# dgrzech/sobfu

Hardware: AMD Instinct MI355X
Metric: solver iterations/sec on 256^3 voxel grid (higher is better)
Workload: dtype f32

## Files before the change

include/sobfu_hip.h:

```cpp
#ifndef SOBFU_HIP_H
#define SOBFU_HIP_H

#include <stddef.h>
#include <stdint.h>

#if defined(__GNUC__)
#pragma GCC visibility push(default)
#endif
#ifdef __cplusplus
extern "C" {
#endif

#define SOBFU_HIP_ABI_VERSION 3

#define SOBFU_E_BADARG (-1)
#define SOBFU_E_FILTER (-2)
#define SOBFU_E_UNSUPPORTED (-3)

int sobfu_hip_abi_version(void);
const char* sobfu_hip_error_string(int code);

int sobfu_hip_clear_volume(float* d_vol, int X, int Y, int Z, void* stream);
int sobfu_hip_integrate_depth(const float* d_dists, int dists_step_bytes, int rows, int cols, float* d_vol, int X,
                              int Y, int Z, const float voxel_size[3], float trunc_dist, float eta,
// ... 10 lines not shown
int sobfu_hip_init_plane(float* d_vol, int X, int Y, int Z, const float voxel_size[3], float trunc_dist, float z,
                         void* stream);
int sobfu_hip_init_torus(float* d_vol, int X, int Y, int Z, const float voxel_size[3], float trunc_dist,
                         const float t[2], void* stream);

int sobfu_hip_bilateral_filter(const uint16_t* d_src, int src_step_bytes, uint16_t* d_dst, int dst_step_bytes,
                               int rows, int cols, int kernel_size, float sigma_spatial, float sigma_depth,
                               void* stream);
int sobfu_hip_truncate_depth(uint16_t* d_depth, int step_bytes, int rows, int cols, float max_dist_m, void* stream);
int sobfu_hip_compute_dists(const uint16_t* d_depth, int depth_step_bytes, float* d_dists, int dists_step_bytes,
                            int rows, int cols, float fx, float fy, float cx, float cy, void* stream);

int sobfu_hip_clear_field(float* d_field, int X, int Y, int Z, void* stream);
int sobfu_hip_init_identity(float* d_psi, int X, int Y, int Z, void* stream);
int sobfu_hip_apply(const float* d_phi, float* d_phi_warped, const float* d_psi, int X, int Y, int Z, void* stream);
int sobfu_hip_estimate_inverse(const float* d_psi, float* d_psi_inv, int X, int Y, int Z, int n_sweeps,
                               void* stream);
int sobfu_hip_inverse_and_warp(const float* d_psi, float* d_psi_inv, const float* d_phi, float* d_phi_warped, int X, int Y, int Z,
                               int n_sweeps, void* stream);
int sobfu_hip_tsdf_gradient(const float* d_vol, float* d_grad, int X, int Y, int Z, void* stream);
int sobfu_hip_laplacian(const float* d_psi, float* d_L, int X, int Y, int Z, void* stream);
int sobfu_hip_jacobian(const float* d_psi, float* d_J, int X, int Y, int Z, int mode, void* stream);
int sobfu_hip_clear_jacobian(float* d_J, int X, int Y, int Z, void* stream);

int sobfu_hip_sobolev_filter(int s, float lambda, float* out);
int sobfu_hip_potential_gradient(const float* d_phi_n_psi, const float* d_phi_global, const float* d_grad,
                                 const float* d_L, float* d_nabla_U, float w_reg, int X, int Y, int Z, void* stream);
int sobfu_hip_convolution_rows(float* d_dst, const float* d_src, const float taps[7], int w, int h, int d,
                               void* stream);
int sobfu_hip_convolution_columns(float* d_dst, const float* d_src, const float taps[7], int w, int h, int d,
                                  void* stream);
int sobfu_hip_convolution_depth(float* d_dst, const float* d_src, const float taps[7], int w, int h, int d,
                                void* stream);
int sobfu_hip_update_psi(float* d_psi, const float* d_nabla_U_S, float* d_updates, float alpha, int X, int Y, int Z,
                         void* stream);

int sobfu_hip_reduce_config(int n, int* blocks, int* threads);
int sobfu_hip_data_energy(const float* d_phi_global, const float* d_phi_n, int n, void* d_scratch, float* out,
                          void* stream);
int sobfu_hip_reg_energy_sobolev(const float* d_J, int n, void* d_scratch, float* out, void* stream);
int sobfu_hip_max_update_norm(const float* d_updates, int n, void* d_scratch, float out[2], void* stream);
int sobfu_hip_reg_energy_sobolev_from_psi(const float* d_psi, int X, int Y, int Z, void* d_scratch, float* out,
                                          void* stream);

int sobfu_hip_fused_potential_gradient(const float* d_phi_n_psi, const float* d_phi_global, const float* d_psi,
                                       float* d_nabla_U, float w_reg, int X, int Y, int Z, void* stream);
int sobfu_hip_fused_smooth_update_apply(const float* d_nabla_U, float* d_psi, const float* d_phi_n,
                                        float* d_phi_n_psi, float* d_updates, uint32_t* d_max_sq_slots,
                                        const float taps[7], float alpha, int X, int Y, int Z, void* stream);

int sobfu_hip_pack_vec3(const float* d_src4, float* d_dst3, size_t n, void* stream);
int sobfu_hip_unpack_vec3(const float* d_src3, float* d_dst4, size_t n, void* stream);
int sobfu_hip_extract_tsdf(const float* d_src2, float* d_dst1, size_t n, void* stream);

int sobfu_hip_tile3_init_identity(float* d_psi, int Lx, int Ly, int Lz, int xb, int yb, int zb, void* stream);
int sobfu_hip_tile3_apply(const float* d_phi, int Xg, int Yg, int Zg, float* d_phi_warped, const float* d_psi, int Lx, int Ly, int Lz,
                          void* stream);
int sobfu_hip_tile3_estimate_inverse(const float* d_psi, int Xg, int Yg, int Zg, float* d_psi_inv, int Lx, int Ly, int Lz, int xb, int yb,
                                     int zb, int n_sweeps, void* stream);
int sobfu_hip_tile3_estimate_inverse_window(const float* d_psi_win, const int win[6], int Xg, int Yg, int Zg, float* d_psi_inv, int Lx, int Ly, int Lz,
                                            int xb, int yb, int zb, const int box[6], int n_sweeps, int* d_violation, void* stream);
int sobfu_hip_tile3_apply_window(const float* d_phi_win, const int win[6], int Xg, int Yg, int Zg, float* d_phi_warped, const float* d_psi, int Lx,
                                 int Ly, int Lz, const int box[6], int* d_violation, void* stream);
int sobfu_hip_tile3_max_displacement(const float* d_psi, int Lx, int Ly, int Lz, int xb, int yb, int zb, const int box[6], uint32_t* d_max_bits,
                                     void* stream);
int sobfu_hip_tile3_integrate_depth(const float* d_dists, int dists_step_bytes, int rows, int cols, float* d_vol_local, int Lx, int Ly,
                                    int Lz, int xb, int yb, int zb, const float voxel_size[3], float trunc_dist, float eta,
                                    const float R[9], const float t[3], float fx, float fy, float cx, float cy, void* stream);
int sobfu_hip_tile3_potential_gradient(const float* d_phi_n_psi, const float* d_phi_global, const float* d_psi, float* d_nabla_U,
                                       float w_reg, int Lx, int Ly, int Lz, const int box[6], int thin,
                                       const uint32_t* d_prev_slots, float max_update_norm, int compact, void* stream);
int sobfu_hip_tile3_smooth_update_apply(const float* d_nabla_U, float* d_psi, const float* d_phi_n, float* d_phi_n_psi, float* d_updates,
                                        uint32_t* d_max_sq_slots, const float taps[7], float alpha, int Lx, int Ly, int Lz, int Xg,
                                        int Yg, int Zg, const int own[6], const int box[6], int thin,
                                        const uint32_t* d_prev_slots, float max_update_norm, int compact, void* stream);
int sobfu_hip_tile3_apply_tsdf_only(const float* d_phi1, int Xg, int Yg, int Zg, float* d_out1, const float* d_psi3, int Lx, int Ly, int Lz,
                                    void* stream);
int sobfu_hip_tile3_pack(const float* d_field3, int Lx, int Ly, int Lz, float* d_buf, const int* boxes, int n_boxes, void* stream);
int sobfu_hip_tile3_unpack(float* d_field3, int Lx, int Ly, int Lz, const float* d_buf, const int* boxes, int n_boxes, void* stream);

typedef struct sobfu_hip_solver sobfu_hip_solver;

typedef struct {
    int verbosity;
    int max_iter;
    int s;
    float max_update_norm;
    float lambda;
    float alpha;
    float w_reg;
} sobfu_hip_solver_params;

typedef struct {
    int iterations;
    int converged;
    float last_max_update_norm;
    float last_max_update_index;
    float last_e_data, last_e_reg;
} sobfu_hip_solver_report;

int sobfu_hip_solver_create(sobfu_hip_solver** out, int X, int Y, int Z, const sobfu_hip_solver_params* params);
int sobfu_hip_solver_destroy(sobfu_hip_solver* s);
int sobfu_hip_solver_set_params(sobfu_hip_solver* s, const sobfu_hip_solver_params* params);
size_t sobfu_hip_solver_workspace_bytes(const sobfu_hip_solver* s);
int sobfu_hip_solver_estimate_psi(sobfu_hip_solver* s, const float* d_phi_global, float* d_phi_global_psi_inv,
                                  const float* d_phi_n, float* d_phi_n_psi, float* d_psi, float* d_psi_inv,
// ... 190 lines not shown
```

sobfu_amd/build_host.py:

```python
from __future__ import annotations

import os
import subprocess

HERE = os.path.dirname(os.path.abspath(__file__))
ROOT = os.path.dirname(HERE)
ROCM = os.environ.get("ROCM_PATH", "/opt/rocm")
INC = os.path.join(ROOT, "include")
CSRC = os.path.join(HERE, "csrc")
LIB = os.path.join(HERE, "libsobfu_hip.so")
SOBFU_HPP = os.path.join(INC, "sobfu_amd", "sobfu.hpp")
DEPTH_IO_HPP = os.path.join(INC, "sobfu_amd", "depth_io.hpp")
SOBFU_HIP_H = os.path.join(INC, "sobfu_hip.h")
EVALUATE_HPP = os.path.join(INC, "sobfu_amd", "evaluate.hpp")


def _test_src(name: str) -> str:
    return os.path.join(ROOT, "tests", "cpp", name)


def _build(out: str, src: str, deps, linked: bool, force: bool = False, flags=()) -> str:
    out = os.path.join(ROOT, "build", out)
    deps = [src, *deps] + ([LIB] if linked else [])
    if not force and os.path.exists(out) and all(os.path.getmtime(out) >= os.path.getmtime(d) for d in deps):
# ... 16 lines not shown
    return _build("depth_io_tool", _test_src("depth_io_tool.cpp"), [DEPTH_IO_HPP], False, force, ["-std=c++14", "-lz"])


def build_png_tool(force: bool = False) -> str:
    return _build("png_write_tool", _test_src("png_write_tool.cpp"), [DEPTH_IO_HPP], False, force, ["-std=c++14", "-lz"])


def build_colour_tool(force: bool = False) -> str:
    return _build("colour_io_tool", _test_src("colour_io_tool.cpp"), [DEPTH_IO_HPP, SOBFU_HPP, SOBFU_HIP_H], True, force)


def build_ply_tool(force: bool = False) -> str:
    return _build("ply_write_tool", _test_src("ply_write_tool.cpp"), [SOBFU_HPP, SOBFU_HIP_H], True, force)


def build_variant_tool(force: bool = False) -> str:
    return _build("variant_tool", _test_src("variant_tool.cpp"), [os.path.join(CSRC, "sobfu_variant.hpp"), SOBFU_HIP_H], False, force,
                  ["-std=c++17", f"-I{CSRC}"])


def build_geometry_tool(force: bool = False, flags=()) -> str:
    deps = [os.path.join(CSRC, h) for h in ("sobfu_geometry.hpp", "sobfu_tile_layout.hpp", "sobfu_variant.hpp")] + [SOBFU_HIP_H]
    return _build("geometry_tool", _test_src("geometry_tool.cpp"), deps, False, force, ["-std=c++17", f"-I{CSRC}", *flags])


def build_icp_tool(force: bool = False) -> str:
    return _build("icp_shell_tool", _test_src("icp_shell_tool.cpp"), [SOBFU_HPP], True, force)


def build_mesh_warp_tool(force: bool = False) -> str:
    return _build("mesh_warp_tool", _test_src("mesh_warp_tool.cpp"), [SOBFU_HPP, DEPTH_IO_HPP], True, force)


def build_mesh_eval_tool(force: bool = False) -> str:
    deps = [SOBFU_HPP, EVALUATE_HPP, SOBFU_HIP_H, os.path.join(CSRC, "sobfu_mesh_distance.hpp")]
    return _build("mesh_eval_tool", _test_src("mesh_eval_tool.cpp"), deps, True, force, [f"-I{CSRC}", "-ffp-contract=off"])


def build_mesh_ray_tool(force: bool = False, flags=()) -> str:
    deps = [os.path.join(CSRC, h) for h in ("sobfu_mesh_ray.hpp", "sobfu_mesh_distance.hpp")]
    return _build("mesh_ray_tool", _test_src("mesh_ray_tool.cpp"), deps, False, force, ["-std=c++14", f"-I{CSRC}", "-ffp-contract=off", *flags])


def build_mesh_parity_tool(force: bool = False, flags=()) -> str:
    deps = [os.path.join(CSRC, h) for h in ("sobfu_mesh_parity.hpp", "sobfu_mesh_distance.hpp")]
    return _build("mesh_parity_tool", _test_src("mesh_parity_tool.cpp"), deps, False, force, ["-std=c++14", f"-I{CSRC}", "-ffp-contract=off", *flags])


def build_rigid_tool(force: bool = False) -> str:
    return _build("rigid_solve_tool", _test_src("rigid_solve_tool.cpp"), [os.path.join(CSRC, "sobfu_rigid.hpp")], False, force,
                  ["-std=c++14", f"-I{CSRC}", "-ffp-contract=off"])


def build_host(force: bool = False) -> str:
    for build in (build_app, build_io_tool, build_png_tool, build_colour_tool, build_ply_tool, build_variant_tool, build_geometry_tool,
                  build_icp_tool, build_mesh_warp_tool, build_mesh_eval_tool, build_mesh_ray_tool, build_mesh_parity_tool, build_rigid_tool):
        build(force)
    return _build("host_shell_tests", _test_src("host_shell_tests.cpp"), [SOBFU_HPP, EVALUATE_HPP, SOBFU_HIP_H], True, force)


if __name__ == "__main__":
    print(build_host(force=True))
```

sobfu_amd/csrc/sobfu_launch.hpp:

```cpp
#pragma once
#include <hip/hip_runtime.h>

#include <cstddef>
#include <cstdint>

#include "sobfu_geometry.hpp"

namespace sobfu_hip {
struct PassALaunch {
    const float* pnp = nullptr;
    const float* pg  = nullptr;
    const float* psi = nullptr;
    float* nU        = nullptr;
    float w_reg      = 0.f;
    int X = 0, Y = 0, Z = 0;
    LaunchBox boxes[kMaxBoxes] = {};
    int n_boxes = 0;
    const uint32_t* prev_slots = nullptr;
    float max_update_norm      = 0.f;
    bool compact = false;
    bool warp    = false;
};
struct PassBLaunch {
    const float* nU     = nullptr;
    float* psi          = nullptr;
    float* psi_out      = nullptr;
    const float* phi_n  = nullptr;
    float* pnp          = nullptr;
    float* updates      = nullptr;
    uint32_t* slots     = nullptr;
    const float* taps   = nullptr;
    float alpha         = 0.f;
    int X = 0, Y = 0, Z = 0;
    int pX = 0, pY = 0, pZ = 0;
    int own[6] = {};
    LaunchBox boxes[kMaxBoxes] = {};
    int n_boxes = 0;
    const uint32_t* prev_slots = nullptr;
    float max_update_norm      = 0.f;
    int prev_rows = 1;
    bool compact  = false;
    bool sys_acquire = false;
    bool warp        = false;
};
inline void set_whole_grid(PassALaunch& l, int X, int Y, int Z) {
    l.X = X; l.Y = Y; l.Z = Z;
    l.boxes[0] = LaunchBox{0, X, 0, Y, 0, Z, false};
    l.n_boxes  = 1;
}
inline void set_whole_grid(PassBLaunch& l, int X, int Y, int Z) {
    l.X = X; l.Y = Y; l.Z = Z;
    l.pX = X; l.pY = Y; l.pZ = Z;
    const int own[6] = {0, X, 0, Y, 0, Z};
    for (int i = 0; i < 6; ++i) l.own[i] = own[i];
    l.boxes[0] = LaunchBox{0, X, 0, Y, 0, Z, false};
    l.n_boxes  = 1;
}
int launch_pass_a(const PassALaunch& l, hipStream_t stream);
int launch_pass_b(const PassBLaunch& l, hipStream_t stream);
constexpr int kMaxSync = 64;
struct TileSync {
    uint32_t ticket_push, reserved;
    uint64_t wait_ticks;
    uint32_t wait_count, pad0;
    uint32_t err;
    uint32_t n_sync;
    uint32_t my_rank, world;
    uint64_t timeout_ticks;
    uint32_t* my_flags;
    uint32_t* my_grows;
    int sync_rank[kMaxSync];
    uint32_t* peer_flags[kMaxSync];
    uint32_t* peer_grows[kMaxSync];
};
struct TilePassAPlan;
int tile_pass_a_plan_create(TilePassAPlan** out, const TileLaunchBox* boxes, int n, int X, int Y, int Z);
void tile_pass_a_plan_destroy(TilePassAPlan* p);
int launch_tile_pass_a_plan(const TilePassAPlan* p, const float* pnp, const float* pg, const float* psi, float* nU, float w_reg, TileSync* sync,
                            uint32_t seq, int wait, const uint32_t* row, uint32_t row_index, hipStream_t stream);
int launch_tile_flush(TileSync* sync, uint32_t seq, int wait, const uint32_t* row, uint32_t row_index, hipStream_t stream);
int launch_tile_pingpong(TileSync* sync, int q, int first, uint32_t seq0, int reps, hipStream_t stream);
int launch_pack_vec(const float* src4, float* dst3, size_t N, hipStream_t stream);
int launch_unpack_vec(const float* src3, float* dst4, size_t N, hipStream_t stream);
int launch_extract_tsdf(const float* src2, float* dst1, size_t N, hipStream_t stream);
int launch_apply_tsdf_only(const float* phi1, float* out1, const float* psi3, int X, int Y, int Z, hipStream_t stream, int phi_Z = 0, int phi_X = 0,
                           int phi_Y = 0);
int launch_msg_copy(bool pack, float* field3, float* buf, int Lx, int Ly, int Lz, const int* boxes, int n, hipStream_t stream);
int launch_msg_scatter_table(float* field3, const float* buf, const uint32_t* d_table, unsigned n_cells, hipStream_t stream);
int launch_compact_enter(const float* psi4, const float* pg2, const float* pn2, float* c_psi, float* c_g, float* c_n, float* c_f, int X, int Y,
                         int Z, hipStream_t stream);
int launch_compact_leave(const float* c_psi, const float* pn2, float* psi4, float* pnp2, int X, int Y, int Z, hipStream_t stream);
int data_energy_tsdf(const float* g1, const float* f1, int n, void* d_scratch, float* out, hipStream_t stream);
int reg_energy_from_psi3(const float* psi3, int X, int Y, int Z, void* d_scratch, float* out, hipStream_t stream);
}
```

sobfu_amd/csrc/sobfu_variant.hpp:

```cpp
#pragma once

#include <cstddef>
#include <cstdlib>

#include "sobfu_hip.h"

namespace sobfu_hip {

inline long env_cache_cells() {
    const char* e = getenv("SOBFU_CACHE_CELLS");
    return e ? atol(e) : 3300000L;
}
inline int env_pipe_b() {
    const char* e = getenv("SOBFU_PIPE_B");
    return e ? (atoi(e) != 0 ? 1 : 0) : -1;
}
inline bool env_warp_a() {
    const char* e = getenv("SOBFU_WARP_A");
    return !(e && atoi(e) == 0);
}

struct GridTraits {
    bool resident;
    bool idx32;
    bool arrays32;
    bool plane32;
    int pipe_b;
};
inline GridTraits grid_traits(int X, int Y, int Z, int pX, int pY, int pZ, long cache_cells, int pipe_b = -1) {
    const size_t n = (size_t) X * Y * Z;
    GridTraits g;
    g.resident = (long) n <= cache_cells;
    g.idx32    = (size_t) pX * pY * pZ < ((size_t) 1 << 30);
    g.arrays32 = n * 12 < ((size_t) 1 << 32);
    g.plane32  = (size_t) X * Y * 16 < ((size_t) 1 << 32);
    g.pipe_b   = pipe_b;
    return g;
}

struct PassAVariant {
    bool compact, nt, warp;
    constexpr bool operator==(const PassAVariant& o) const { return compact == o.compact && nt == o.nt && warp == o.warp; }
};
inline constexpr PassAVariant kPassATable[] = {
    {true,      true,  true},
    {true,      false, false},
    {true,      true,  false},
    {false,     false, false},
};
inline constexpr PassAVariant kTilePassATable[] = {
    {true,  false, false},
    {true,  true,  false},
    {false, false, false},
};
inline int choose_pass_a(const GridTraits& g, bool compact, bool warp, bool tile, PassAVariant* v) {
    if (warp && (tile || !compact || g.resident || !g.idx32)) return SOBFU_E_UNSUPPORTED;
    v->compact = compact;
    v->nt      = compact && !g.resident;
    v->warp    = warp;
    return 0;
}

struct PassBVariant {
    bool updates, compact, direct, idx32, lead, nt, pipe, ntbuf, apply;
    constexpr bool operator==(const PassBVariant& o) const {
        return updates == o.updates && compact == o.compact && direct == o.direct && idx32 == o.idx32 && lead == o.lead && nt == o.nt &&
               pipe == o.pipe && ntbuf == o.ntbuf && apply == o.apply;
    }
};
inline constexpr PassBVariant kPassBTable[] = {
    {true , true , true , false, false, true , false, false, true },
// ... 13 lines not shown
    {false, true , false, true , true , true , false, false, true },
    {false, true , false, true , false, false, true , false, true },
    {false, true , false, true , false, false, false, false, true },
    {false, true , false, true , false, true , true , false, true },
    {false, true , false, true , false, true , false, true , true },
    {false, true , false, true , false, true , false, false, true },
    {false, true , false, false, false, true , false, false, true },
    {false, false, false, false, false, true , false, false, true },
};
struct PassBAsk {
    bool compact, updates;
    bool sys_acquire;
    bool apply;
};
struct PassBMarch {
    bool pipe         = false;
    bool direct       = false;
    bool long_marches = false;
};
inline int pass_b_march(const GridTraits& g, const PassBAsk& k, PassBMarch* m) {
    if (!g.plane32) return SOBFU_E_UNSUPPORTED;
    if (k.sys_acquire && !g.arrays32) return SOBFU_E_UNSUPPORTED;
    m->pipe = k.compact && g.idx32 && !k.updates && g.arrays32 && (k.sys_acquire || (g.pipe_b >= 0 ? g.pipe_b != 0 : g.resident));
    if (k.sys_acquire && !m->pipe) return SOBFU_E_UNSUPPORTED;
    return 0;
}
inline int choose_pass_b(const GridTraits& g, const PassBAsk& k, const PassBMarch& m, PassBVariant* v) {
    if (!k.apply && (m.direct || !k.compact || !g.idx32 || k.updates || g.resident || m.pipe || !g.arrays32 || k.sys_acquire))
        return SOBFU_E_UNSUPPORTED;
    const bool own_format = k.compact && g.idx32 && !k.updates, plain_nt = !g.resident && !m.pipe;
    v->updates = k.updates;
    v->compact = k.compact;
    v->direct  = m.direct;
    v->idx32   = own_format;
    v->lead    = own_format && plain_nt && !m.direct && m.long_marches;
    v->nt      = !own_format || !g.resident;
    v->pipe    = own_format && m.pipe;
    v->ntbuf   = own_format && plain_nt && g.arrays32;
    v->apply   = k.apply;
    return 0;
}

inline bool loop_warps_in_pass_a(const GridTraits& g) {
    const PassBAsk b{true, false, false, false};
    PassAVariant va;
    PassBVariant vb;
    PassBMarch m;
    return choose_pass_a(g, true, true, false, &va) == 0 && pass_b_march(g, b, &m) == 0 && choose_pass_b(g, b, m, &vb) == 0;
}
inline bool loop_warps_in_pass_a(int X, int Y, int Z) {
    return env_warp_a() && loop_warps_in_pass_a(grid_traits(X, Y, Z, X, Y, Z, env_cache_cells(), env_pipe_b()));
}

}
```

sobfu_amd/csrc/solver_capi.hip:

```cpp
#include <algorithm>
#include <cmath>
#include <cstdio>
#include <cstdlib>
#include <cstring>
#include <string>
#include <vector>

#include "sobfu_device.hpp"
#include "sobfu_hip.h"
#include "sobfu_host.hpp"
#include "sobfu_launch.hpp"


namespace {

using sobfu_hip::DevicePtr;
using sobfu_hip::EventPtr;
using sobfu_hip::kSlots;
using sobfu_hip::slots_to_norm;
constexpr int kCheckEvery = 32;
constexpr int kMaxRunAhead = 96;

}

struct sobfu_hip_solver {
    int X = 0, Y = 0, Z = 0;
    size_t N = 0;
    sobfu_hip_solver_params p{};
    float taps[7]{};
    DevicePtr<float> nabla_U;
    DevicePtr<float> updates;
    DevicePtr<float> c_psi;
    DevicePtr<float> c_f;
    DevicePtr<float> c_g;
    DevicePtr<float> c_n;
    bool compact = true;
    DevicePtr<uint32_t> slots;
    sobfu_hip::PinnedPtr<uint32_t> h_rows;
    int h_rows_iters   = 0;
    EventPtr ev_chk;
    DevicePtr<void> red_scratch;
    int slots_iters    = 0;
    bool keep_updates  = false;
    sobfu_hip_log_fn log_fn = nullptr;
    void* log_user          = nullptr;
    bool log_set            = false;
    size_t bytes            = 0;
    int prof_stride = 0;
    std::vector<EventPtr> events;
    double ms_a = 0, ms_b = 0;
    int prof_launches = 0, prof_pending = 0;
    struct Session {
        bool active = false, compact = false;
        const float *pg = nullptr, *pn = nullptr;
        float *pnp = nullptr, *psi = nullptr;
        const float *it_pnp = nullptr, *it_pg = nullptr, *it_pn = nullptr;
        float *it_psi = nullptr, *it_out = nullptr, *upd = nullptr;
        int cap = 0;
        int launched = 0;
        int checked = 0, fl_to = 0;
        bool in_flight = false;
        int done = 0;
        bool converged = false;
        float last_norm = 0.f;
        bool inline_log = false;
        bool warp = false;
    } q;

    void log(const std::string& line) const {
        if (log_set) {
            if (log_fn) log_fn(line.c_str(), log_user);
        } else {
            std::printf("%s\n", line.c_str());
        }
    }
};

namespace {

std::string fmt_g(float v) {
    char b[64];
    std::snprintf(b, sizeof b, "%g", (double) v);
    return b;
}

int ensure_slots(sobfu_hip_solver* s, int iters) {
    if (iters <= s->slots_iters) return 0;
    if (s->slots) s->bytes -= (size_t) (s->slots_iters + 1) * kSlots * 4;
    s->slots_iters = 0;
    SOBFU_HIP_TRY(sobfu_hip::device_alloc(s->slots, (size_t) (iters + 1) * kSlots * 4));
    s->slots_iters = iters;
    s->bytes += (size_t) (iters + 1) * kSlots * 4;
    return 0;
}

int ensure_poll(sobfu_hip_solver* s, int iters) {
    if (!s->ev_chk) SOBFU_HIP_TRY(sobfu_hip::event_create(s->ev_chk, hipEventDisableTiming));
    if (iters <= s->h_rows_iters) return 0;
    s->h_rows.reset();
    s->h_rows_iters = 0;
    void* h = nullptr;
    SOBFU_HIP_TRY(hipHostMalloc(&h, (size_t) iters * kSlots * 4, hipHostMallocDefault));
    s->h_rows.reset((uint32_t*) h);
    s->h_rows_iters = iters;
    return 0;
}

int ensure_compact(sobfu_hip_solver* s) {
    if (s->c_psi) return 0;
    SOBFU_HIP_TRY(sobfu_hip::device_alloc(s->c_psi, s->N * 12));
    SOBFU_HIP_TRY(sobfu_hip::device_alloc(s->c_f, s->N * 4));
    SOBFU_HIP_TRY(sobfu_hip::device_alloc(s->c_g, s->N * 4));
    SOBFU_HIP_TRY(sobfu_hip::device_alloc(s->c_n, s->N * 4));
    s->bytes += s->N * 24;
    return 0;
}

int ensure_updates(sobfu_hip_solver* s) {
    if (s->updates) return 0;
    SOBFU_HIP_TRY(sobfu_hip::device_alloc(s->updates, s->N * 16));
    s->bytes += s->N * 16;
    return 0;
}

int set_params(sobfu_hip_solver* s, const sobfu_hip_solver_params* p) {
    SOBFU_CHECK_ARGS(p && p->max_iter >= 0);
    if (p->s < 7 || p->s > 16) return p->s < 7 ? SOBFU_E_UNSUPPORTED : SOBFU_E_FILTER;
    float h[16];
    SOBFU_TRY(sobfu_hip_sobolev_filter(p->s, p->lambda, h));
    for (int i = 0; i < 7; ++i) s->taps[i] = h[i];
    s->p = *p;
    return 0;
}

int ensure_events(sobfu_hip_solver* s, size_t n) {
    while (s->events.size() < n) {
        EventPtr e;
        SOBFU_HIP_TRY(sobfu_hip::event_create(e, hipEventDefault));
        s->events.push_back(std::move(e));
    }
    return 0;
}

int session_begin_impl(sobfu_hip_solver* s, const float* pg, const float* pn, float* pnp, float* psi, int cap, hipStream_t st) {
    sobfu_hip_solver::Session& q = s->q;
    const int X = s->X, Y = s->Y, Z = s->Z;
    q = sobfu_hip_solver::Session{};
    q.pg = pg; q.pn = pn; q.pnp = pnp; q.psi = psi;
    q.cap = cap;
    q.compact = s->compact && cap > 0;
    q.last_norm = NAN;
    if (!q.compact) SOBFU_TRY(sobfu_hip_apply(pn, pnp, psi, X, Y, Z, st));
    if (cap <= 0) return 0;
    SOBFU_TRY(ensure_slots(s, cap));
    SOBFU_HIP_TRY(hipMemsetAsync(s->slots.get(), 0, (size_t) (cap + 1) * kSlots * 4, st));
    if (s->keep_updates) {
        SOBFU_TRY(ensure_updates(s));
        q.upd = s->updates.get();
    }
    q.it_pnp = pnp; q.it_pg = pg; q.it_pn = pn; q.it_psi = psi; q.it_out = pnp;
    if (q.compact) {
        SOBFU_TRY(ensure_compact(s));
        SOBFU_TRY(sobfu_hip::launch_compact_enter(psi, pg, pn, s->c_psi.get(), s->c_g.get(), s->c_n.get(), s->c_f.get(), X, Y, Z, st));
        q.it_pnp = s->c_f.get(); q.it_pg = s->c_g.get(); q.it_pn = s->c_n.get(); q.it_psi = s->c_psi.get(); q.it_out = s->c_f.get();
        q.warp = s->p.verbosity == 0 && !q.upd && sobfu_hip::loop_warps_in_pass_a(X, Y, Z);
    }
    if (s->p.max_update_norm >= 0.f) SOBFU_TRY(ensure_poll(s, cap));
    if (s->prof_stride > 0) SOBFU_TRY(ensure_events(s, (size_t) 3 * (cap / s->prof_stride + 1)));
    return 0;
}
int session_begin(sobfu_hip_solver* s, const float* pg, const float* pn, float* pnp, float* psi, int cap, hipStream_t st) {
    if (s->q.active) return SOBFU_E_BADARG;
    const int rc = session_begin_impl(s, pg, pn, pnp, psi, cap, st);
    s->q.active = rc == 0;
    return rc;
}

void session_examine(sobfu_hip_solver* s, int upto, float* per_iter) {
    sobfu_hip_solver::Session& q = s->q;
    for (int k = q.checked; k < upto && !q.converged; ++k) {
        const float v = slots_to_norm(s->h_rows.get() + (size_t) k * kSlots);
        if (per_iter) per_iter[k] = v;
        q.last_norm = v;
        q.done = k + 1;
        if (v <= s->p.max_update_norm) q.converged = true;
    }
    q.checked = upto;
}

int session_enqueue(sobfu_hip_solver* s, int n, bool poll, float* per_iter, hipStream_t st) {
    sobfu_hip_solver::Session& q = s->q;
    if (!q.active || n < 0 || q.launched + n > q.cap) return SOBFU_E_BADARG;
    const int X = s->X, Y = s->Y, Z = s->Z;
    const sobfu_hip_solver_params& p = s->p;
    const bool can_converge = p.max_update_norm >= 0.f;
    const int last = q.launched + n;
    sobfu_hip::PassALaunch A;
    sobfu_hip::set_whole_grid(A, X, Y, Z);
    A.pnp = q.warp ? q.it_pn : q.it_pnp; A.pg = q.it_pg; A.psi = q.it_psi; A.nU = s->nabla_U.get(); A.w_reg = p.w_reg;
    A.max_update_norm = p.max_update_norm;
    A.compact = q.compact;
    A.warp    = q.warp;
    sobfu_hip::PassBLaunch B;
    sobfu_hip::set_whole_grid(B, X, Y, Z);
    B.nU = s->nabla_U.get(); B.psi = q.it_psi; B.phi_n = q.it_pn; B.pnp = q.it_out; B.updates = q.upd; B.taps = s->taps; B.alpha = p.alpha;
    B.max_update_norm = p.max_update_norm;
    B.compact = q.compact;
    B.warp    = q.warp;
    for (int it = q.launched + 1; it <= last && !q.converged; ++it) {
        const uint32_t* prev = (it > 1) ? s->slots.get() + (size_t) (it - 1) * kSlots : nullptr;
        uint32_t* cur        = s->slots.get() + (size_t) it * kSlots;
        const bool ev = s->prof_stride > 0 && (it % s->prof_stride == 0) && (size_t) 3 * (s->prof_pending + 1) <= s->events.size();
        const int e0  = 3 * s->prof_pending;
        if (ev) SOBFU_HIP_TRY(hipEventRecord(s->events[e0].get(), st));
        A.prev_slots = B.prev_slots = prev;
        B.slots = cur;
        SOBFU_TRY(sobfu_hip::launch_pass_a(A, st));
        if (ev) SOBFU_HIP_TRY(hipEventRecord(s->events[e0 + 1].get(), st));
        SOBFU_TRY(sobfu_hip::launch_pass_b(B, st));
        if (ev) {
            SOBFU_HIP_TRY(hipEventRecord(s->events[e0 + 2].get(), st));
            s->prof_pending += 1;
        }
        q.launched = it;
        if (can_converge && poll) {
            if (!q.in_flight && (it % kCheckEvery == 0 || it == last)) {
                SOBFU_HIP_TRY(hipMemcpyAsync(s->h_rows.get() + (size_t) q.checked * kSlots, s->slots.get() + (size_t) (q.checked + 1) * kSlots,
                                             (size_t) (it - q.checked) * kSlots * 4, hipMemcpyDeviceToHost, st));
                SOBFU_HIP_TRY(hipEventRecord(s->ev_chk.get(), st));
                q.in_flight = true;
                q.fl_to     = it;
            }
            if (q.in_flight) {
                const bool must_wait = it - q.checked >= kMaxRunAhead;
                hipError_t e = must_wait ? hipEventSynchronize(s->ev_chk.get()) : hipEventQuery(s->ev_chk.get());
                if (e == hipSuccess) {
                    session_examine(s, q.fl_to, per_iter);
                    q.in_flight = false;
                } else if (e != hipErrorNotReady) {
                    return (int) e;
                }
            }
        }
    }
    return 0;
}

int session_drain(sobfu_hip_solver* s, float* per_iter, hipStream_t st) {
    sobfu_hip_solver::Session& q = s->q;
    if (q.launched == 0) return 0;
    if (s->p.max_update_norm >= 0.f) {
        if (q.in_flight) {
            SOBFU_HIP_TRY(hipEventSynchronize(s->ev_chk.get()));
            session_examine(s, q.fl_to, per_iter);
            q.in_flight = false;
// ... 301 lines not shown
```

sobfu_amd/csrc/solver_kernels.hip:

```cpp
#include <type_traits>

#include "sobfu_device.hpp"
#include "sobfu_hip.h"
#include "sobfu_host.hpp"
#include "sobfu_launch.hpp"

using namespace sobfu_hip;

#ifndef SOBFU_SWIZZLE_B
#define SOBFU_SWIZZLE_B true
#endif

namespace {

struct Taps {
    float s[7];
};
constexpr int kMaxMsgs = 18;

#include "solver_iter_common.inl"
#include "solver_pass_a.inl"
#include "solver_pass_b.inl"
#include "solver_aux_kernels.inl"

}

namespace sobfu_hip {

template <size_t I = 0, class Row, size_t N, class F>
static bool launch_row(const Row (&table)[N], const Row& v, F&& launch) {
    if constexpr (I < N) {
        if (table[I] == v) {
            launch(std::integral_constant<size_t, I>{});
            return true;
        }
        return launch_row<I + 1>(table, v, launch);
    } else {
        return false;
    }
}

static int launch_tile_boxes(const TilePassAArgsP& a, int groups, const PassAVariant& v, hipStream_t stream) {
    const dim3 grid((unsigned) groups), block(TX, kWY);
    const bool found = launch_row(kTilePassATable, v, [&](auto i) {
        constexpr PassAVariant V = kTilePassATable[decltype(i)::value];
        hipLaunchKernelGGL((tile_potential_gradient_kernel<kRPT, kWY, V.compact, V.nt ? kNT : 0>), grid, block, 0, stream, a);
    });
    return found ? (int) hipGetLastError() : SOBFU_E_UNSUPPORTED;
}

int launch_pass_a(const PassALaunch& L, hipStream_t stream) {
    if (L.n_boxes > kMaxBoxes) return SOBFU_E_BADARG;
    const bool direct = has_direct_box(L.boxes, L.n_boxes);
    const GridTraits g = grid_traits(L.X, L.Y, L.Z, L.X, L.Y, L.Z, env_cache_cells());
    PassAVariant v;
    SOBFU_TRY(choose_pass_a(g, L.compact, L.warp, direct, &v));
    if (direct) {
        TileBoxList B{};
        const int total = plan_pass_a_thin(B, L.boxes, L.n_boxes, g.resident);
        if (total <= 0) return total < 0 ? SOBFU_E_BADARG : 0;
        TileBoxList* d = nullptr;
        SOBFU_HIP_TRY(hipMallocAsync((void**) &d, sizeof B, stream));
        const hipError_t e = hipMemcpyAsync(d, &B, sizeof B, hipMemcpyHostToDevice, stream);
        const TilePassAArgsP a{{L.pnp, L.pg, L.psi, L.nU, {L.X, L.Y, L.Z}, L.w_reg, nullptr, 0.f}, d, {nullptr, 0, 0, nullptr, 0}};
        const int rc = e != hipSuccess ? (int) e : launch_tile_boxes(a, total, v, stream);
        const hipError_t f = hipFreeAsync(d, stream);
        return rc != 0 ? rc : (int) f;
    }
    PassAArgs a{{L.pnp, L.pg, L.psi, L.nU, {L.X, L.Y, L.Z}, L.w_reg, L.prev_slots, L.max_update_norm}, {}};
    const int groups = plan_pass_a(a.boxes, L.boxes, L.n_boxes);
    if (groups == 0) return 0;
    const dim3 grid((unsigned) groups), block(TX, kWY);
    const bool found = launch_row(kPassATable, v, [&](auto i) {
        constexpr PassAVariant V = kPassATable[decltype(i)::value];
        hipLaunchKernelGGL((fused_potential_gradient_kernel<kRPT, kWY, V.compact, V.nt ? kNT : 0, V.warp>), grid, block, 0, stream, a);
    });
    return found ? (int) hipGetLastError() : SOBFU_E_UNSUPPORTED;
}

struct TilePassAPlan {
    TileBoxList* d_boxes = nullptr;
    int groups = 0, X = 0, Y = 0, Z = 0;
};
int tile_pass_a_plan_create(TilePassAPlan** out, const TileLaunchBox* boxes, int n, int X, int Y, int Z) {
    TileBoxList L{};
    const int total = fill_tile_boxes(L, boxes, n, grid_traits(X, Y, Z, X, Y, Z, env_cache_cells()).resident);
    if (total < 0) return SOBFU_E_BADARG;
    auto* p = new TilePassAPlan();
    p->groups = total; p->X = X; p->Y = Y; p->Z = Z;
    hipError_t e = hipSuccess;
    if (total > 0) {
        e = hipMalloc((void**) &p->d_boxes, sizeof L);
        if (e == hipSuccess) e = hipMemcpy(p->d_boxes, &L, sizeof L, hipMemcpyHostToDevice);
    }
    if (e != hipSuccess) {
        if (p->d_boxes) (void) hipFree(p->d_boxes);
        delete p;
        return (int) e;
    }
    *out = p;
    return 0;
}
void tile_pass_a_plan_destroy(TilePassAPlan* p) {
    if (p == nullptr) return;
    if (p->d_boxes) (void) hipFree(p->d_boxes);
    delete p;
}
int launch_tile_pass_a_plan(const TilePassAPlan* p, const float* pnp, const float* pg, const float* psi, float* nU, float w_reg, TileSync* sync,
                            uint32_t seq, int wait, const uint32_t* row, uint32_t row_index, hipStream_t stream) {
    if (p->groups == 0) return 0;
    PassAVariant v;
    SOBFU_TRY(choose_pass_a(grid_traits(p->X, p->Y, p->Z, p->X, p->Y, p->Z, env_cache_cells()), true, false, true, &v));
    const TilePassAArgsP a{{pnp, pg, psi, nU, {p->X, p->Y, p->Z}, w_reg, nullptr, 0.f}, p->d_boxes, {sync, seq, wait, row, row_index}};
    return launch_tile_boxes(a, p->groups, v, stream);
}

int launch_tile_pingpong(TileSync* sync, int q, int first, uint32_t seq0, int reps, hipStream_t stream) {
    hipLaunchKernelGGL(tile_pingpong_kernel, dim3(1), dim3(64), 0, stream, sync, q, first, seq0, reps);
    return (int) hipGetLastError();
}

int launch_tile_flush(TileSync* sync, uint32_t seq, int wait, const uint32_t* row, uint32_t row_index, hipStream_t stream) {
    hipLaunchKernelGGL(tile_flush_kernel, dim3(1), dim3(64), 0, stream, sync, seq, wait, row, row_index);
    return (int) hipGetLastError();
}

int launch_pass_b(const PassBLaunch& L, hipStream_t stream) {
    if (L.n_boxes > kMaxBoxes) return SOBFU_E_BADARG;
// ... 64 lines not shown
    return (int) hipGetLastError();
}
#undef SOBFU_LIN
int launch_compact_enter(const float* psi4, const float* pg2, const float* pn2, float* c_psi, float* c_g, float* c_n, float* c_f, int X, int Y,
                         int Z, hipStream_t stream) {
    hipLaunchKernelGGL(compact_enter_kernel, voxel_grid(X, Y, Z), voxel_block(), 0, stream, (const float4*) psi4, (const float2*) pg2,
                       (const float2*) pn2, (P3*) c_psi, c_g, c_n, c_f, Dims{X, Y, Z});
    return (int) hipGetLastError();
}
int launch_compact_leave(const float* c_psi, const float* pn2, float* psi4, float* pnp2, int X, int Y, int Z, hipStream_t stream) {
    hipLaunchKernelGGL(compact_leave_kernel, voxel_grid(X, Y, Z), voxel_block(), 0, stream, (const P3*) c_psi, (const float2*) pn2,
                       (float4*) psi4, (float2*) pnp2, Dims{X, Y, Z});
    return (int) hipGetLastError();
}

}

extern "C" {

int sobfu_hip_fused_potential_gradient(const float* d_phi_n_psi, const float* d_phi_global, const float* d_psi,
                                       float* d_nabla_U, float w_reg, int X, int Y, int Z, void* stream) {
    SOBFU_CHECK_ARGS(d_phi_n_psi && d_phi_global && d_psi && d_nabla_U && X > 1 && Y > 1 && Z > 1);
    if ((size_t) X * Y * Z > (size_t) 0x7fffffff) return SOBFU_E_UNSUPPORTED;
    sobfu_hip::PassALaunch L;
    sobfu_hip::set_whole_grid(L, X, Y, Z);
    L.pnp = d_phi_n_psi; L.pg = d_phi_global; L.psi = d_psi; L.nU = d_nabla_U; L.w_reg = w_reg;
    return sobfu_hip::launch_pass_a(L, (hipStream_t) stream);
}

int sobfu_hip_fused_smooth_update_apply(const float* d_nabla_U, float* d_psi, const float* d_phi_n, float* d_phi_n_psi,
                                        float* d_updates, uint32_t* d_max_sq_slots, const float taps[7], float alpha,
                                        int X, int Y, int Z, void* stream) {
    SOBFU_CHECK_ARGS(d_nabla_U && d_psi && d_phi_n && d_phi_n_psi && d_max_sq_slots && taps && X > 0 && Y > 0 && Z > 0);
    if ((size_t) X * Y * Z > (size_t) 0x7fffffff) return SOBFU_E_UNSUPPORTED;
    sobfu_hip::PassBLaunch L;
    sobfu_hip::set_whole_grid(L, X, Y, Z);
    L.nU = d_nabla_U; L.psi = d_psi; L.phi_n = d_phi_n; L.pnp = d_phi_n_psi; L.updates = d_updates; L.slots = d_max_sq_slots;
    L.taps = taps; L.alpha = alpha;
    return sobfu_hip::launch_pass_b(L, (hipStream_t) stream);
}

int sobfu_hip_pack_vec3(const float* d_src4, float* d_dst3, size_t n, void* stream) {
    SOBFU_CHECK_ARGS(d_src4 && d_dst3 && n > 0);
    return sobfu_hip::launch_pack_vec(d_src4, d_dst3, n, (hipStream_t) stream);
}
int sobfu_hip_unpack_vec3(const float* d_src3, float* d_dst4, size_t n, void* stream) {
    SOBFU_CHECK_ARGS(d_src3 && d_dst4 && n > 0);
    return sobfu_hip::launch_unpack_vec(d_src3, d_dst4, n, (hipStream_t) stream);
}
int sobfu_hip_extract_tsdf(const float* d_src2, float* d_dst1, size_t n, void* stream) {
    SOBFU_CHECK_ARGS(d_src2 && d_dst1 && n > 0);
    return sobfu_hip::launch_extract_tsdf(d_src2, d_dst1, n, (hipStream_t) stream);
}
static bool box_ok(const int b[6], int Lx, int Ly, int Lz) {
    return b[0] >= 0 && b[0] <= b[1] && b[1] <= Lx && b[2] >= 0 && b[2] <= b[3] && b[3] <= Ly && b[4] >= 0 && b[4] <= b[5] && b[5] <= Lz;
}

int sobfu_hip_tile3_potential_gradient(const float* d_phi_n_psi, const float* d_phi_global, const float* d_psi, float* d_nabla_U, float w_reg,
                                       int Lx, int Ly, int Lz, const int box[6], int thin, const uint32_t* d_prev_slots,
                                       float max_update_norm, int compact, void* stream) {
    SOBFU_CHECK_ARGS(d_phi_n_psi && d_phi_global && d_psi && d_nabla_U && Lx > 1 && Ly > 1 && Lz > 1 && box && box_ok(box, Lx, Ly, Lz));
    if ((size_t) Lx * Ly * Lz > (size_t) 0x7fffffff) return SOBFU_E_UNSUPPORTED;
    sobfu_hip::PassALaunch L;
    L.pnp = d_phi_n_psi; L.pg = d_phi_global; L.psi = d_psi; L.nU = d_nabla_U; L.w_reg = w_reg;
    L.X = Lx; L.Y = Ly; L.Z = Lz;
    L.boxes[0] = sobfu_hip::LaunchBox{box[0], box[1], box[2], box[3], box[4], box[5], thin != 0};
    L.n_boxes = 1;
    L.prev_slots = d_prev_slots; L.max_update_norm = max_update_norm;
    L.compact = compact != 0;
    return sobfu_hip::launch_pass_a(L, (hipStream_t) stream);
}

int sobfu_hip_tile3_smooth_update_apply(const float* d_nabla_U, float* d_psi, const float* d_phi_n, float* d_phi_n_psi, float* d_updates,
                                        uint32_t* d_max_sq_slots, const float taps[7], float alpha, int Lx, int Ly, int Lz, int Xg, int Yg,
                                        int Zg, const int own[6], const int box[6], int thin, const uint32_t* d_prev_slots,
                                        float max_update_norm, int compact, void* stream) {
    SOBFU_CHECK_ARGS(d_nabla_U && d_psi && d_phi_n && d_phi_n_psi && d_max_sq_slots && taps && Lx > 0 && Ly > 0 && Lz > 0 && Xg > 0 && Yg > 0 &&
                     Zg > 0 && own && box && box_ok(own, Lx, Ly, Lz) && box_ok(box, Lx, Ly, Lz));
    if ((size_t) Lx * Ly * Lz > (size_t) 0x7fffffff || (size_t) Xg * Yg * Zg > (size_t) 0x7fffffff) return SOBFU_E_UNSUPPORTED;
    sobfu_hip::PassBLaunch L;
    L.nU = d_nabla_U; L.psi = d_psi; L.phi_n = d_phi_n; L.pnp = d_phi_n_psi; L.updates = d_updates; L.slots = d_max_sq_slots;
    L.taps = taps; L.alpha = alpha;
    L.X = Lx; L.Y = Ly; L.Z = Lz;
    L.pX = Xg; L.pY = Yg; L.pZ = Zg;
    for (int i = 0; i < 6; ++i) L.own[i] = own[i];
    L.boxes[0] = sobfu_hip::LaunchBox{box[0], box[1], box[2], box[3], box[4], box[5], thin != 0};
    L.n_boxes = 1;
    L.prev_slots = d_prev_slots; L.max_update_norm = max_update_norm;
    L.compact = compact != 0;
    return sobfu_hip::launch_pass_b(L, (hipStream_t) stream);
}

int sobfu_hip_tile3_apply_tsdf_only(const float* d_phi1, int Xg, int Yg, int Zg, float* d_out1, const float* d_psi3, int Lx, int Ly, int Lz,
                                    void* stream) {
    SOBFU_CHECK_ARGS(d_phi1 && d_out1 && d_psi3 && Lx > 0 && Ly > 0 && Lz > 0 && Xg > 0 && Yg > 0 && Zg > 0);
    return sobfu_hip::launch_apply_tsdf_only(d_phi1, d_out1, d_psi3, Lx, Ly, Lz, (hipStream_t) stream, Zg, Xg, Yg);
}

int sobfu_hip_tile3_pack(const float* d_field3, int Lx, int Ly, int Lz, float* d_buf, const int* boxes, int n_boxes, void* stream) {
    SOBFU_CHECK_ARGS(d_field3 && d_buf && boxes && n_boxes >= 0 && Lx > 0 && Ly > 0 && Lz > 0);
    return sobfu_hip::launch_msg_copy(true, const_cast<float*>(d_field3), d_buf, Lx, Ly, Lz, boxes, n_boxes, (hipStream_t) stream);
}

int sobfu_hip_tile3_unpack(float* d_field3, int Lx, int Ly, int Lz, const float* d_buf, const int* boxes, int n_boxes, void* stream) {
    SOBFU_CHECK_ARGS(d_field3 && d_buf && boxes && n_boxes >= 0 && Lx > 0 && Ly > 0 && Lz > 0);
    return sobfu_hip::launch_msg_copy(false, d_field3, const_cast<float*>(d_buf), Lx, Ly, Lz, boxes, n_boxes, (hipStream_t) stream);
// ... 4 lines not shown
```

sobfu_amd/ops.py:

```python
from __future__ import annotations

import ctypes as C

import numpy as np
import torch

from . import _lib
from ._lib import SolverParams, SolverReport, check

_F3 = C.c_float * 3
_F2 = C.c_float * 2
_F7 = C.c_float * 7
_F9 = C.c_float * 9


def _require_gpu():
    if not torch.cuda.is_available():
        raise RuntimeError("sobfu_amd needs a HIP device (MI355X); there is no CPU fallback")


def _ptr(t: torch.Tensor, dtype=torch.float32):
    if not (t.is_cuda and t.is_contiguous() and t.dtype == dtype):
        raise ValueError(f"expected a contiguous {dtype} tensor on the GPU, got {t.dtype} {t.device} contiguous={t.is_contiguous()}")
    return C.c_void_p(t.data_ptr())
# ... 186 lines not shown
    check(_lib.lib().sobfu_hip_reduce_config(C.c_int(n), C.byref(b), C.byref(t)), "reduce_config")
    return b.value, t.value


def _scratch(dev):
    return torch.empty(65536 * 2, dtype=torch.float32, device=dev)


def data_energy(phi_global, phi_n):
    out, sc = C.c_float(), _scratch(phi_global.device)
    check(_lib.lib().sobfu_hip_data_energy(_ptr(phi_global), _ptr(phi_n), C.c_int(phi_global.numel() // 2), _ptr(sc),
                                           C.byref(out), _stream()), "data_energy")
    return out.value


def reg_energy_sobolev(J):
    out, sc = C.c_float(), _scratch(J.device)
    check(_lib.lib().sobfu_hip_reg_energy_sobolev(_ptr(J), C.c_int(J.numel() // 16), _ptr(sc), C.byref(out), _stream()),
          "reg_energy_sobolev")
    return out.value


def reg_energy_sobolev_from_psi(psi):
    out, sc = C.c_float(), _scratch(psi.device)
    check(_lib.lib().sobfu_hip_reg_energy_sobolev_from_psi(_ptr(psi), *_xyz(psi), _ptr(sc), C.byref(out), _stream()),
          "reg_energy_sobolev_from_psi")
    return out.value


def max_update_norm(updates):
    out, sc = _F2(), _scratch(updates.device)
    check(_lib.lib().sobfu_hip_max_update_norm(_ptr(updates), C.c_int(updates.numel() // 4), _ptr(sc), out, _stream()),
          "max_update_norm")
    return out[0], out[1]


def fused_potential_gradient(phi_n_psi, phi_global, psi, nabla_U, w_reg):
    check(_lib.lib().sobfu_hip_fused_potential_gradient(_ptr(phi_n_psi), _ptr(phi_global), _ptr(psi), _ptr(nabla_U),
                                                        _f(w_reg), *_xyz(psi), _stream()), "fused_potential_gradient")


def fused_smooth_update_apply(nabla_U, psi, phi_n, phi_n_psi, S, alpha, updates=None, slots=None):
    if slots is None:
        slots = torch.zeros(256, dtype=torch.int32, device=psi.device)
    up = _ptr(updates) if updates is not None else None
    check(_lib.lib().sobfu_hip_fused_smooth_update_apply(_ptr(nabla_U), _ptr(psi), _ptr(phi_n), _ptr(phi_n_psi), up,
                                                         _ptr(slots, torch.int32), _taps(S), _f(alpha), *_xyz(psi),
                                                         _stream()), "fused_smooth_update_apply")
    m = np.float32(slots.max().cpu().numpy().view(np.float32))
    r = np.sqrt(m, dtype=np.float32)
    if r > 0 and np.float64(r) * np.float64(r) > np.float64(m):
        r = np.nextafter(r, np.float32(-np.inf), dtype=np.float32)
    return float(r)


class Solver:

    def __init__(self, dims, *, max_iter, alpha, w_reg, s=7, lam=0.1, max_update_norm=-1.0, verbosity=0, quiet=True):
        _require_gpu()
        self.dims = tuple(int(d) for d in dims)
        self.params = SolverParams(verbosity, max_iter, s, max_update_norm, np.float32(lam), alpha, w_reg)
        self._h = C.c_void_p()
        check(_lib.lib().sobfu_hip_solver_create(C.byref(self._h), *[C.c_int(d) for d in self.dims],
                                                 C.byref(self.params)), "solver_create")
        self.log_lines = []
        self._cb = _lib.LOG_FN(self._on_log)
        self._quiet = quiet
        check(_lib.lib().sobfu_hip_solver_set_logger(self._h, self._cb, None), "solver_set_logger")

    def _on_log(self, line, _user):
        self.log_lines.append(line.decode())
        if not self._quiet:
            print(line.decode())

    def close(self):
        if getattr(self, "_h", None):
            _lib.lib().sobfu_hip_solver_destroy(self._h)
            self._h = None

    __del__ = close

    def workspace_bytes(self):
        return int(_lib.lib().sobfu_hip_solver_workspace_bytes(self._h))

    def set_compact(self, enable=True):
        check(_lib.lib().sobfu_hip_solver_set_compact(self._h, C.c_int(1 if enable else 0)), "set_compact")

    def set_profiling(self, stride=1):
        check(_lib.lib().sobfu_hip_solver_set_profiling(self._h, C.c_int(int(stride))), "set_profiling")

    def get_profile(self, reset=True):
        a, b, n = C.c_float(), C.c_float(), C.c_int()
        check(_lib.lib().sobfu_hip_solver_get_profile(self._h, C.byref(a), C.byref(b), C.byref(n), C.c_int(1 if reset else 0)),
              "get_profile")
        return a.value, b.value, n.value

    def keep_updates(self, keep=True):
        check(_lib.lib().sobfu_hip_solver_keep_updates(self._h, C.c_int(1 if keep else 0)), "keep_updates")

    def updates(self):
        p = _lib.lib().sobfu_hip_solver_updates(self._h)
        if not p:
            raise _lib.HipError("solver_updates: allocation failed")
        X, Y, Z = self.dims

        class _Raw:
# ... 600 lines not shown
```

Baseline: 4444.

## Precompute flat-brick mask of phi_n to let pass A skip uniform bricks

Adds a kernel that classifies bricks (edge 8/16/32) of the compacted phi_n TSDF and writes a bitmask (packed 16 bricks per word, so two bits per brick, apparently more than a flat/non-flat flag). The solver builds this mask once per solve when the warp pass-A variant is active, and passes it to the fused potential-gradient kernel. The kernel can then take a cheaper path in bricks where the field is flat, for example truncated regions with zero gradient. It adds a small allocation and one pre-pass kernel. Correctness depends on the kernel's flatness test being exact. The kernel bodies (flat_bricks_kernel, FlatBricks, PassAWarpArgs handling) are not visible here.

```diff
diff --git a/include/sobfu_hip.h b/include/sobfu_hip.h
--- a/include/sobfu_hip.h
+++ b/include/sobfu_hip.h
@@ -86,6 +86,9 @@
 int sobfu_hip_pack_vec3(const float* d_src4, float* d_dst3, size_t n, void* stream);
 int sobfu_hip_unpack_vec3(const float* d_src3, float* d_dst4, size_t n, void* stream);
 int sobfu_hip_extract_tsdf(const float* d_src2, float* d_dst1, size_t n, void* stream);
+
+int sobfu_hip_flat_brick_edge(int X, int Y, int Z);
+int sobfu_hip_flat_bricks(const float* d_tsdf1, int X, int Y, int Z, int edge, uint32_t* d_mask, void* stream);
 
 int sobfu_hip_tile3_init_identity(float* d_psi, int Lx, int Ly, int Lz, int xb, int yb, int zb, void* stream);
 int sobfu_hip_tile3_apply(const float* d_phi, int Xg, int Yg, int Zg, float* d_phi_warped, const float* d_psi, int Lx, int Ly, int Lz,
diff --git a/sobfu_amd/build_host.py b/sobfu_amd/build_host.py
--- a/sobfu_amd/build_host.py
+++ b/sobfu_amd/build_host.py
@@ -92,9 +92,15 @@
                   ["-std=c++14", f"-I{CSRC}", "-ffp-contract=off"])
 
 
+def build_flat_tool(force: bool = False) -> str:
+    return _build("flat_bricks_tool", _test_src("flat_bricks_tool.cpp"), [os.path.join(CSRC, "sobfu_variant.hpp"), SOBFU_HIP_H], False, force,
+                  ["-std=c++17", f"-I{CSRC}", "-ffp-contract=off", "-fopenmp"])
+
+
 def build_host(force: bool = False) -> str:
     for build in (build_app, build_io_tool, build_png_tool, build_colour_tool, build_ply_tool, build_variant_tool, build_geometry_tool,
-                  build_icp_tool, build_mesh_warp_tool, build_mesh_eval_tool, build_mesh_ray_tool, build_mesh_parity_tool, build_rigid_tool):
+                  build_icp_tool, build_mesh_warp_tool, build_mesh_eval_tool, build_mesh_ray_tool, build_mesh_parity_tool, build_rigid_tool,
+                  build_flat_tool):
         build(force)
     return _build("host_shell_tests", _test_src("host_shell_tests.cpp"), [SOBFU_HPP, EVALUATE_HPP, SOBFU_HIP_H], True, force)
 
diff --git a/sobfu_amd/csrc/sobfu_launch.hpp b/sobfu_amd/csrc/sobfu_launch.hpp
--- a/sobfu_amd/csrc/sobfu_launch.hpp
+++ b/sobfu_amd/csrc/sobfu_launch.hpp
@@ -20,7 +20,10 @@
     float max_update_norm      = 0.f;
     bool compact = false;
     bool warp    = false;
+    const uint32_t* flat_mask = nullptr;
+    int flat_edge             = 0;
 };
+constexpr size_t kFlatMapBytes = 8192;
 struct PassBLaunch {
     const float* nU     = nullptr;
     float* psi          = nullptr;
@@ -90,6 +93,7 @@
 int launch_compact_enter(const float* psi4, const float* pg2, const float* pn2, float* c_psi, float* c_g, float* c_n, float* c_f, int X, int Y,
                          int Z, hipStream_t stream);
 int launch_compact_leave(const float* c_psi, const float* pn2, float* psi4, float* pnp2, int X, int Y, int Z, hipStream_t stream);
+int launch_flat_bricks(const float* tsdf1, int X, int Y, int Z, int edge, uint32_t* mask, hipStream_t stream);
 int data_energy_tsdf(const float* g1, const float* f1, int n, void* d_scratch, float* out, hipStream_t stream);
 int reg_energy_from_psi3(const float* psi3, int X, int Y, int Z, void* d_scratch, float* out, hipStream_t stream);
 }
diff --git a/sobfu_amd/csrc/sobfu_variant.hpp b/sobfu_amd/csrc/sobfu_variant.hpp
--- a/sobfu_amd/csrc/sobfu_variant.hpp
+++ b/sobfu_amd/csrc/sobfu_variant.hpp
@@ -17,6 +17,10 @@
 }
 inline bool env_warp_a() {
     const char* e = getenv("SOBFU_WARP_A");
+    return !(e && atoi(e) == 0);
+}
+inline bool env_flat_a() {
+    const char* e = getenv("SOBFU_FLAT_A");
     return !(e && atoi(e) == 0);
 }
 
@@ -136,4 +140,14 @@
     return env_warp_a() && loop_warps_in_pass_a(grid_traits(X, Y, Z, X, Y, Z, env_cache_cells(), env_pipe_b()));
 }
 
+constexpr int kFlatBricks = 32768;
+inline int flat_brick_edge(int X, int Y, int Z) {
+    if (X <= 0 || Y <= 0 || Z <= 0) return 0;
+    for (int e = 8; e <= 32; e *= 2) {
+        const size_t n = (size_t) ((X + e - 1) / e) * (size_t) ((Y + e - 1) / e) * (size_t) ((Z + e - 1) / e);
+        if (n <= (size_t) kFlatBricks) return e;
+    }
+    return 0;
 }
+
+}
diff --git a/sobfu_amd/csrc/solver_capi.hip b/sobfu_amd/csrc/solver_capi.hip
--- a/sobfu_amd/csrc/solver_capi.hip
+++ b/sobfu_amd/csrc/solver_capi.hip
@@ -34,6 +34,7 @@
     DevicePtr<float> c_f;
     DevicePtr<float> c_g;
     DevicePtr<float> c_n;
+    DevicePtr<uint32_t> flat;
     bool compact = true;
     DevicePtr<uint32_t> slots;
     sobfu_hip::PinnedPtr<uint32_t> h_rows;
@@ -65,6 +66,8 @@
         float last_norm = 0.f;
         bool inline_log = false;
         bool warp = false;
+        const uint32_t* flat = nullptr;
+        int flat_edge = 0;
     } q;
 
     void log(const std::string& line) const {
@@ -113,6 +116,13 @@
     SOBFU_HIP_TRY(sobfu_hip::device_alloc(s->c_g, s->N * 4));
     SOBFU_HIP_TRY(sobfu_hip::device_alloc(s->c_n, s->N * 4));
     s->bytes += s->N * 24;
+    return 0;
+}
+
+int ensure_flat(sobfu_hip_solver* s) {
+    if (s->flat) return 0;
+    SOBFU_HIP_TRY(sobfu_hip::device_alloc(s->flat, sobfu_hip::kFlatMapBytes));
+    s->bytes += sobfu_hip::kFlatMapBytes;
     return 0;
 }
 
@@ -164,6 +174,12 @@
         SOBFU_TRY(sobfu_hip::launch_compact_enter(psi, pg, pn, s->c_psi.get(), s->c_g.get(), s->c_n.get(), s->c_f.get(), X, Y, Z, st));
         q.it_pnp = s->c_f.get(); q.it_pg = s->c_g.get(); q.it_pn = s->c_n.get(); q.it_psi = s->c_psi.get(); q.it_out = s->c_f.get();
         q.warp = s->p.verbosity == 0 && !q.upd && sobfu_hip::loop_warps_in_pass_a(X, Y, Z);
+        const int edge = q.warp && sobfu_hip::env_flat_a() ? sobfu_hip::flat_brick_edge(X, Y, Z) : 0;
+        if (edge > 0) {
+            SOBFU_TRY(ensure_flat(s));
+            SOBFU_TRY(sobfu_hip::launch_flat_bricks(s->c_n.get(), X, Y, Z, edge, s->flat.get(), st));
+            q.flat = s->flat.get(); q.flat_edge = edge;
+        }
     }
     if (s->p.max_update_norm >= 0.f) SOBFU_TRY(ensure_poll(s, cap));
     if (s->prof_stride > 0) SOBFU_TRY(ensure_events(s, (size_t) 3 * (cap / s->prof_stride + 1)));
@@ -201,6 +217,7 @@
     A.max_update_norm = p.max_update_norm;
     A.compact = q.compact;
     A.warp    = q.warp;
+    A.flat_mask = q.flat; A.flat_edge = q.flat_edge;
     sobfu_hip::PassBLaunch B;
     sobfu_hip::set_whole_grid(B, X, Y, Z);
     B.nU = s->nabla_U.get(); B.psi = q.it_psi; B.phi_n = q.it_pn; B.pnp = q.it_out; B.updates = q.upd; B.taps = s->taps; B.alpha = p.alpha;
diff --git a/sobfu_amd/csrc/solver_kernels.hip b/sobfu_amd/csrc/solver_kernels.hip
--- a/sobfu_amd/csrc/solver_kernels.hip
+++ b/sobfu_amd/csrc/solver_kernels.hip
@@ -47,6 +47,24 @@
         hipLaunchKernelGGL((tile_potential_gradient_kernel<kRPT, kWY, V.compact, V.nt ? kNT : 0>), grid, block, 0, stream, a);
     });
     return found ? (int) hipGetLastError() : SOBFU_E_UNSUPPORTED;
+}
+
+static bool flat_geometry(int X, int Y, int Z, int edge, int* shift, int* nbx, int* nby, int* nb) {
+    if (edge != 8 && edge != 16 && edge != 32) return false;
+    *shift = edge == 8 ? 3 : edge == 16 ? 4 : 5;
+    *nbx   = (X + edge - 1) / edge;
+    *nby   = (Y + edge - 1) / edge;
+    const size_t n = (size_t) *nbx * (size_t) *nby * (size_t) ((Z + edge - 1) / edge);
+    if (n > (size_t) kFlatBricks) return false;
+    *nb = (int) n;
+    return true;
+}
+static_assert(kFlatBricks == 16 * kFlatWords && kFlatMapBytes == 4 * kFlatWords, "the map's sizes: bricks, words, bytes");
+int launch_flat_bricks(const float* tsdf1, int X, int Y, int Z, int edge, uint32_t* mask, hipStream_t stream) {
+    int shift, nbx, nby, nb;
+    if (!flat_geometry(X, Y, Z, edge, &shift, &nbx, &nby, &nb)) return SOBFU_E_BADARG;
+    hipLaunchKernelGGL(flat_bricks_kernel, dim3((unsigned) ((nb + 15) / 16)), dim3(256), 0, stream, tsdf1, Dims{X, Y, Z}, shift, nbx, nby, nb, mask);
+    return (int) hipGetLastError();
 }
 
 int launch_pass_a(const PassALaunch& L, hipStream_t stream) {
@@ -68,12 +86,19 @@
         return rc != 0 ? rc : (int) f;
     }
     PassAArgs a{{L.pnp, L.pg, L.psi, L.nU, {L.X, L.Y, L.Z}, L.w_reg, L.prev_slots, L.max_update_norm}, {}};
+    FlatBricks flat{nullptr, 0, 0, 0, 0};
+    if (L.warp && L.flat_mask != nullptr) {
+        int shift, nbx, nby, nb;
+        if (!flat_geometry(L.X, L.Y, L.Z, L.flat_edge, &shift, &nbx, &nby, &nb)) return SOBFU_E_BADARG;
+        flat = FlatBricks{L.flat_mask, shift, nbx, nby, (nb + 15) / 16};
+    }
     const int groups = plan_pass_a(a.boxes, L.boxes, L.n_boxes);
     if (groups == 0) return 0;
     const dim3 grid((unsigned) groups), block(TX, kWY);
     const bool found = launch_row(kPassATable, v, [&](auto i) {
         constexpr PassAVariant V = kPassATable[decltype(i)::value];
-        hipLaunchKernelGGL((fused_potential_gradient_kernel<kRPT, kWY, V.compact, V.nt ? kNT : 0, V.warp>), grid, block, 0, stream, a);
+        if constexpr (V.warp) hipLaunchKernelGGL((fused_potential_gradient_kernel<kRPT, kWY, V.compact, V.nt ? kNT : 0, true>), grid, block, 0, stream, PassAWarpArgs{a.c, a.boxes, flat});
+        else hipLaunchKernelGGL((fused_potential_gradient_kernel<kRPT, kWY, V.compact, V.nt ? kNT : 0, false>), grid, block, 0, stream, a);
     });
     return found ? (int) hipGetLastError() : SOBFU_E_UNSUPPORTED;
 }
@@ -244,6 +269,12 @@
     SOBFU_CHECK_ARGS(d_src2 && d_dst1 && n > 0);
     return sobfu_hip::launch_extract_tsdf(d_src2, d_dst1, n, (hipStream_t) stream);
 }
+int sobfu_hip_flat_brick_edge(int X, int Y, int Z) { return sobfu_hip::flat_brick_edge(X, Y, Z); }
+int sobfu_hip_flat_bricks(const float* d_tsdf1, int X, int Y, int Z, int edge, uint32_t* d_mask, void* stream) {
+    SOBFU_CHECK_ARGS(d_tsdf1 && d_mask && X > 0 && Y > 0 && Z > 0);
+    if ((size_t) X * Y * Z > (size_t) 0x7fffffff) return SOBFU_E_UNSUPPORTED;
+    return sobfu_hip::launch_flat_bricks(d_tsdf1, X, Y, Z, edge, d_mask, (hipStream_t) stream);
+}
 static bool box_ok(const int b[6], int Lx, int Ly, int Lz) {
     return b[0] >= 0 && b[0] <= b[1] && b[1] <= Lx && b[2] >= 0 && b[2] <= b[3] && b[3] <= Ly && b[4] >= 0 && b[4] <= b[5] && b[5] <= Lz;
 }
diff --git a/sobfu_amd/ops.py b/sobfu_amd/ops.py
--- a/sobfu_amd/ops.py
+++ b/sobfu_amd/ops.py
@@ -262,6 +262,21 @@
     if r > 0 and np.float64(r) * np.float64(r) > np.float64(m):
         r = np.nextafter(r, np.float32(-np.inf), dtype=np.float32)
     return float(r)
+
+
+def flat_brick_edge(dims):
+    X, Y, Z = dims
+    return int(_lib.lib().sobfu_hip_flat_brick_edge(C.c_int(X), C.c_int(Y), C.c_int(Z)))
+
+
+def flat_bricks(tsdf, edge, mask=None):
+    Z, Y, X = tsdf.shape
+    nb = -(-X // edge) * -(-Y // edge) * -(-Z // edge)
+    if mask is None:
+        mask = torch.empty((nb + 15) // 16, dtype=torch.int32, device=tsdf.device)
+    check(_lib.lib().sobfu_hip_flat_bricks(_ptr(tsdf), C.c_int(X), C.c_int(Y), C.c_int(Z), C.c_int(edge), _ptr(mask, torch.int32), _stream()),
+          "flat_bricks")
+    return mask
 
 
 class Solver:
```

New measurement: 4680, median of 3. 1.05x the previous value.
